# gercap/gr-ofdm_tools

Hardware: AMD Instinct MI355X
Metric: IQ Msamples/s Welch-PSD (4096-pt, 50% ovlp) (higher is better)
Workload: dtype f32; 1 GPU; C2: 2^28-sample complex64 stream, 4096-pt Hann Welch, 50% overlap, detrend constant, density; nfft=4096, noverlap=2048, window=hann, samples_per_gpu=268435456, segments_per_gpu=131071, parallelism=single GPU

## Files before the change

gr-ofdm_tools_amd/csrc/abi_route.hip:

```cpp
#include "abi_state.h"


namespace {
constexpr long long kFdMinSegments = 8;

const W4096Variant kVariants[] = {
    {"dpp", launch_welch_tuned4096_dpp, tuned4096_blocks_per_cu_dpp, 8, false},
    {"pipe", launch_welch_tuned4096_pipe, tuned4096_blocks_per_cu_pipe, 16, false},
    {"ws", launch_welch_tuned4096_ws, tuned4096_blocks_per_cu_ws, 20, true, true},
};
const W4096Variant *variant_by_tag(const char *tag) {
    for (const auto &v : kVariants)
        if (!strcmp(v.tag, tag)) return &v;
    return &kVariants[0];
}
const W4096Variant *w4096_variant(int step, bool fd_ok, const std::string &want) {
    const W4096Variant *const dpp = variant_by_tag("dpp"), *const pipe = variant_by_tag("pipe"), *const ws = variant_by_tag("ws");
    const W4096Variant *pick = (step == 2048) ? (fd_ok ? ws : pipe) : dpp;
    if (!want.empty())
        for (const auto &v : kVariants)
            if (want == v.tag) pick = &v;
    if (pick->fd && !fd_ok) pick = pipe;
    if (pick != dpp && step != 2048) pick = dpp;
    return pick;
}

const char *const kRecipeKernelName[] = {"welch_generic", "welch4096", "csd4096", "csd4096ws", "welch16k", "welch16k1x",
                                         "welch16k1x_half", "seg", "segws", "seg_padded", "anyfft"};

int table_bpc(const OccupancyKey &k) {
    switch (k.kern) {
        case RK_W4096: return !strcmp(k.variant, "ws") ? 2 : 4;
        case RK_CSD4096: return 3;
        case RK_CSD4096WS: return 1;
        case RK_SEGWS: return k.nfft == 1024 ? 8 : 4;
        case RK_SEG: {
            const int tpw = k.nfft == 256 ? 4 : (k.nfft == 512 ? 2 : 1), wpt = k.nfft <= 1024 ? 1 : k.nfft / 1024;
            return 4 * (k.seg_wps4 ? 4 : 3) * tpw / wpt;
        }
        case RK_SEGPAD:
            return k.nfft == 1024 ? 16 : (k.nperseg * 4 == k.nfft ? 8 : (k.seg_kind == 0 ? 6 : 8));
        case RK_W16K: case RK_W16K1X: case RK_W16K1X_HALF: return k.nfft == 8192 && !k.half_ws ? 2 : 1;
        default: return 0;
    }
}

int generic_wg_for(int cu_count, int nfft, long long nseg, int nstreams) {
    const size_t lds = generic_lds_bytes(nfft);
    long long occ = (long long)(160 * 1024 / lds);
    const long long tocc = 2048 / generic_threads_for(nfft);
    if (occ > tocc) occ = tocc;
    if (occ < 1) occ = 1;
    if (occ > 4) occ = 4;
    long long w = ((long long)cu_count * occ + nstreams - 1) / nstreams;
    if (w > nseg) w = nseg;
    if (w < 1) w = 1;
    return (int)w;
}
}

namespace oth {
const char *const kAnyKindName[] = {"none", "direct", "twolevel", "bluestein", "bluestein2"};

bool w4096_variant_known(const char *tag) {
    for (const auto &v : kVariants)
        if (!strcmp(tag, v.tag)) return true;
    return false;
}

int runtime_bpc(const OccupancyKey &k) {
    switch (k.kern) {
        case RK_W4096: return variant_by_tag(k.variant)->blocks_per_cu();
        case RK_CSD4096: return csd4096_blocks_per_cu();
        case RK_CSD4096WS: return csd4096ws_blocks_per_cu();
// ... 232 lines not shown
```

gr-ofdm_tools_amd/csrc/abi_state.h:

```cpp
#pragma once
#include "../../include/ofdm_tools_hip.h"
#include "oth_internal.h"
#include "abi_barrier.h"

#include <algorithm>
#include <cmath>
#include <cstdio>
#include <cstdlib>
#include <cstring>
#include <map>
#include <mutex>
#include <new>
#include <string>
#include <vector>

using namespace oth;

struct oth_ctx {
    int device = 0;
    hipStream_t stream = nullptr;
    bool own_stream = false;
    int cu_count = 256;
    std::string err;
    std::string name;
    bool timing = false;
    std::vector<std::pair<hipEvent_t, hipEvent_t>> events;
    std::vector<std::pair<hipEvent_t, hipEvent_t>> free_events;
    double total_ms = 0.0;
    uint64_t launches = 0;
    std::map<int, float2 *> twiddles;
    float *sink = nullptr;
    double *acc4 = nullptr;
    unsigned *queue = nullptr;
    unsigned *done_count = nullptr;
    std::recursive_mutex mu;
    bool queue_clean = false;
    int queue_used = 0;
    unsigned char *scratch = nullptr;
    size_t scratch_cap = 0;
    std::vector<int> bounds_host;
    int *d_bounds = nullptr;
    int *h_bounds = nullptr;
    size_t bounds_cap = 0;
    hipEvent_t bounds_ev = nullptr;
};

struct AnyTables {
    AnyShape sh{};
    const float2 *tw = nullptr;
    float2 *chirp = nullptr;
    float2 *midtab = nullptr;
    float2 *ws = nullptr;
    size_t ws_cap = 0;
    float4 *mean = nullptr;
    size_t mean_cap = 0;
};

struct oth_plan {
    oth_ctx *ctx = nullptr;
    int nfft = 0, nperseg = 0, noverlap = 0, step = 0, detrend = 0, scaling = 0, fftshift = 0, trim = 0;
    int db = 0, kernel = OTH_KERNEL_AUTO, sched = OTH_SCHED_DYNAMIC;
    double fs = 1.0, scale = 1.0;
    float *d_win = nullptr;
    const float2 *d_tw = nullptr;
    float4 *d_fd = nullptr;
    float4 *d_fd1x = nullptr;
    float2 *d_pilot = nullptr;
    size_t pilot_cap = 0;
    bool fast_detrend = false;
    bool rect_window = false;
    float *d_partial = nullptr;
    size_t partial_cap = 0;
    float *d_reduce = nullptr;
    size_t reduce_cap = 0;
    float *d_out = nullptr;
    size_t out_cap = 0;
    static constexpr int kOutRing = 4;
    float *h_out = nullptr;
    unsigned *h_seq = nullptr;
    uint64_t out_ticket[kOutRing] = {0, 0, 0, 0};
    uint64_t out_nseg[kOutRing] = {0, 0, 0, 0};
    uint64_t next_out_ticket = 1;
    bool pilot_launch = false;
    std::string last_recipe;
    float2 *d_stage = nullptr;
    size_t stage_cap = 0;
    float *d_sum = nullptr;
    float *d_wpm = nullptr;
    uint64_t nseg_total = 0;
    size_t carry = 0;
    float2 *d_stream = nullptr;
    size_t stream_cap = 0;
    std::string tune_variant;
    int tune_sched = -1, tune_chunk = 0, tune_tail = 0;
    void *h_ring[4] = {nullptr, nullptr, nullptr, nullptr};
    size_t h_ring_cap[4] = {0, 0, 0, 0};
    hipEvent_t h_ring_ev[4] = {nullptr, nullptr, nullptr, nullptr};
    unsigned h_ring_next = 0;
    AnyTables any;
    std::mutex exec_mu;
    int hostwait = 0;
    int average = OTH_AVERAGE_MEAN;
    float *d_rows = nullptr;
    size_t rows_cap = 0;
    float *d_med = nullptr;
    size_t med_cap = 0;
    unsigned *d_msel = nullptr;
    size_t msel_cap = 0;
    AnyTables rows_any;
    long long bias_nseg = 0;
    double bias = 1.0;
};

struct oth_chain {
    oth_ctx *ctx = nullptr;
    int nfft = 0, fftshift = 0, epilogue = 0, keep_n = 1, count = 1;
    float *d_win = nullptr;
    const float2 *d_tw = nullptr;
    float2 *d_buf = nullptr;
    size_t buf_cap = 0;
    size_t leftover = 0;
    float *d_rows = nullptr;
    size_t rows_cap = 0;
// ... 228 lines not shown
```

gr-ofdm_tools_amd/csrc/abi_welch.hip:

```cpp
#include "abi_state.h"

#include <sched.h>
#include <time.h>

namespace {
bool window_spectrum(const std::vector<float> &w, int n, int band, std::vector<double> &re, std::vector<double> &im) {
    re.assign(n, 0.0);
    im.assign(n, 0.0);
    double s2 = 0.0;
    for (int i = 0; i < n; ++i) {
        re[i] = (double)w[i];
        s2 += (double)w[i] * (double)w[i];
    }
    host_fft_pow2(re, im);
    for (int k = band; k < n - band; ++k)
        if (re[k] * re[k] + im[k] * im[k] > 1e-10 * s2) return false;
    return true;
}

bool window_spectrum_table(const std::vector<float> &w, std::vector<float> &fd) {
    std::vector<double> re, im;
    if (!window_spectrum(w, 4096, 256, re, im)) return false;
    fd.resize(4 * 256);
    for (int t = 0; t < 256; ++t) {
// ... 4 lines not shown
        fd[4 * t + 3] = (float)im[k + 3840];
    }
    return true;
}

bool window_spectrum_table_seg(const std::vector<float> &w, int n, std::vector<float> &fd) {
    const int R = n / 256, Q = 16 / R;
    std::vector<double> re, im;
    if (!window_spectrum(w, n, 256, re, im)) return false;
    fd.assign((size_t)4 * (n / 16) * Q, 0.f);
    for (int t = 0; t < n / 16; ++t) {
        const int k0 = t / R, j = t % R;
        for (int m = 0; m < Q; ++m) {
            const int lo = k0 + 16 * (j + R * m), hi = lo + 256 * (R - 1);
            float *o = &fd[4 * ((size_t)Q * t + m)];
            o[0] = (float)re[lo];
            o[1] = (float)im[lo];
            o[2] = (float)re[hi];
            o[3] = (float)im[hi];
        }
    }
    return true;
}

bool window_spectrum_table_16k(const std::vector<float> &w, int n, std::vector<float> &fd) {
    const int F = n / 4096;
    std::vector<double> re, im;
    if (!window_spectrum(w, n, 256 * F, re, im)) return false;
    fd.assign((size_t)4 * 256 * F, 0.f);
    for (int tid = 0; tid < 256 * F; ++tid) {
        const int kp = tid >> 8, k0 = (tid >> 4) & 15, k1 = tid & 15;
        const int lo = kp + F * (k0 + 16 * k1), hi = kp + F * (k0 + 16 * k1 + 3840);
        fd[4 * tid] = (float)re[lo];
        fd[4 * tid + 1] = (float)im[lo];
        fd[4 * tid + 2] = (float)re[hi];
        fd[4 * tid + 3] = (float)im[hi];
    }
    return true;
}

bool window_spectrum_table_1x(const std::vector<float> &w, int n, std::vector<float> &fd) {
    std::vector<double> re, im;
    if (!window_spectrum(w, n, 16, re, im)) return false;
    fd.assign((size_t)4 * (n / 16), 0.f);
    for (int k0 = 0; k0 < 16; ++k0) {
        const int lo = n == 16384 ? 64 * k0 : 64 * (k0 >> 1) + 32 * (k0 & 1);
        const int hi = n == 16384 ? 64 * k0 + 63 : 64 * (k0 >> 1) + 32 * (k0 & 1) + 31;
        fd[4 * lo] = (float)re[k0];
        fd[4 * lo + 1] = (float)im[k0];
        const int kh = n - 16 + k0;
        fd[4 * hi + 2] = (float)(-im[kh]);
        fd[4 * hi + 3] = (float)re[kh];
    }
    return true;
}

int segments(const oth_plan *p, size_t nsamples, long long *nseg) {
    if (nsamples < (size_t)p->nperseg) return OTH_ERR_INVALID;
    *nseg = (long long)((nsamples - (size_t)p->noverlap) / (size_t)p->step);
    return OTH_OK;
}

int run_average(oth_plan *p, const float2 *x, const float2 *y, size_t nsamples, int nstreams, size_t stride,
                long long *nseg_out, int *W_out, int *layout_out) {
    oth_ctx *c = p->ctx;
    long long nseg = 0;
    if (segments(p, nsamples, &nseg) != OTH_OK)
        return fail(c, OTH_ERR_INVALID, "input shorter than nperseg");
    const bool csd = (y != nullptr);
    LaunchRecipe r;
    const char *why = "";
    if (int rrc = resolve_recipe(shape_of(p), csd, nseg, nstreams, c->cu_count, runtime_bpc, &r, &why))
        return fail(c, rrc, why);
    p->last_recipe = recipe_text(r, p->nfft);
    int rc = ensure(c, &p->d_partial, &p->partial_cap, sizeof(float) * (size_t)nstreams * r.W * r.nch * p->nfft);
    {
        const int groups = std::max(kReduceGroups, finalize_row_groups(p->nfft, r.W, r.nch));
        if (!rc) rc = ensure(c, &p->d_reduce, &p->reduce_cap, sizeof(float) * (size_t)nstreams * groups * r.nch * p->nfft);
    }
    if (rc) return rc;
    const float4 *fd_tab = r.form == 2 ? (r.use_fd1x ? p->d_fd1x : p->d_fd) : nullptr;
    const float2 *pilot = nullptr;
    if (r.pilot == 1) {
        rc = ensure(c, &p->d_pilot, &p->pilot_cap, sizeof(float2) * 2 * kPilotProbes * (size_t)nstreams);
        if (rc) return rc;
        HIPCHK(c, launch_pilot_mean(x, csd ? y : nullptr, stride, p->nperseg, p->step, nseg, nstreams, p->d_pilot, c->stream));
        pilot = p->d_pilot;
    }
    unsigned *queue = nullptr;
    if (r.tickets) {
        queue = c->queue;
        if (!c->queue_clean) HIPCHK(c, hipMemsetAsync(c->queue, 0, sizeof(unsigned) * 64, c->stream));
        c->queue_clean = false;
        c->queue_used = nstreams;
    }
    if (r.kern == RK_ANY && r.any_onewg) {
        Timed tm(c);
        for (int st = 0; st < nstreams; ++st) {
            W32kArgs a{};
            a.x = x + (size_t)st * stride;
            a.first = 0, a.step = p->step, a.nseg = nseg;
            a.win = p->d_win, a.tw = p->any.tw;
            a.partial = p->d_partial + (size_t)st * r.W * p->nfft;
            a.detrend = p->detrend != OTH_DETREND_NONE;
            a.front = p->nfft == 65536, a.wpm = p->d_wpm;
            HIPCHK(c, launch_welch32k(a, r.W, c->stream));
// ... 5 lines not shown
                         p->detrend != OTH_DETREND_NONE, nseg, p->d_partial + (size_t)st * r.W * r.nch * p->nfft, r.W, nullptr, 0,
                         1.0f, 0, p->tune_variant == "anycov");
            if (rc) return rc;
        }
    } else if (r.kern == RK_SEG || r.kern == RK_SEGWS || r.kern == RK_SEGPAD) {
        SegArgs g{};
        g.x = x;
        g.stream_stride = stride;
        g.nstreams = nstreams;
        g.win = p->d_win;
        g.tw = p->d_tw;
        g.first = 0;
        g.step = p->step;
        g.nseg = nseg;
        g.detrend = p->detrend;
        g.chain = 0;
        g.partial = p->d_partial;
        g.wg_per_stream = r.W;
        g.sched = r.sched;
        g.chunk = r.chunk;
        g.tail_chunk = r.tail_chunk;
        g.nbig = r.nbig;
        g.queue = queue;
        g.fd = fd_tab;
        g.pilot = pilot;
        Timed tm(c);
        switch (r.kern) {
            case RK_SEGPAD: HIPCHK(c, launch_seg_padded(p->nfft, p->nperseg, g, r.seg_kind, c->stream)); break;
            case RK_SEGWS: HIPCHK(c, launch_segws(p->nfft, g, r.seg_det, c->stream)); break;
            default: HIPCHK(c, launch_seg(p->nfft, g, r.seg_kind, r.seg_wps4, c->stream)); break;
        }
    } else {
        WelchArgs a;
        a.x = x;
        a.y = y;
        a.win = p->d_win;
        a.tw = p->d_tw;
        a.partial = p->d_partial;
        a.nseg = nseg;
        a.stream_stride = stride;
        a.nperseg = p->nperseg;
        a.step = p->step;
        a.detrend = p->detrend;
        a.wg_per_stream = r.W;
        a.nstreams = nstreams;
        a.sched = r.sched;
        a.chunk = r.chunk;
        a.tail_chunk = r.tail_chunk;
        a.nbig = r.nbig;
        a.queue = queue;
        a.fd = fd_tab;
        a.pilot = pilot;
        a.pilot_inline = r.pilot == 2 ? 1 : 0;
        Timed tm(c);
        switch (r.kern) {
            case RK_W4096: HIPCHK(c, r.variant->launch(a, c->stream)); break;
            case RK_CSD4096WS: HIPCHK(c, launch_csd_tuned4096ws(a, c->stream)); break;
            case RK_CSD4096: HIPCHK(c, launch_csd_tuned4096(a, c->stream)); break;
            case RK_W16K1X_HALF:
                HIPCHK(c, r.half_ws ? launch_welch_tuned8kws(a, c->stream) : launch_welch_tuned16k1x_half(p->nfft, a, c->stream));
                break;
            case RK_W16K1X: HIPCHK(c, launch_welch_tuned16k1x(p->nfft, a, r.x1_window, r.x1_plain, c->stream)); break;
            case RK_W16K: HIPCHK(c, launch_welch_tuned16k(p->nfft, a, c->stream)); break;
            default: HIPCHK(c, launch_welch_generic(p->nfft, a, c->stream)); break;
        }
    }
    *nseg_out = nseg;
    *W_out = r.W;
    *layout_out = r.layout;
    return OTH_OK;
}

int finalize_and_rearm(oth_ctx *c, FinalizeArgs &f, int nstreams) {
    f.queue_reset = nullptr;
    f.queue_n = 0;
    if (!c->queue_clean && c->queue_used > 0) {
        f.queue_reset = c->queue;
        f.queue_n = c->queue_used;
    }
    HIPCHK(c, launch_finalize(f, nstreams, c->stream));
    if (f.queue_reset) {
        c->queue_clean = true;
        c->queue_used = 0;
    }
    return OTH_OK;
}

FinalizeArgs finalize_args(const oth_plan *p, int W, int layout, int nch) {
    FinalizeArgs f{};
    f.partial = p->d_partial;
    f.scratch = p->d_reduce;
    f.W = W;
    f.nfft = p->nfft;
    f.nch = nch;
    f.layout = layout;
    f.l1 = p->any.sh.L1, f.l2 = p->any.sh.L2;
    return f;
}

template <typename P> hipError_t upload_table(oth_ctx *c, P **dst, const std::vector<float> &h) {
    hipError_t e = hipMalloc(dst, sizeof(float) * h.size());
    if (e == hipSuccess) e = hipMemcpyAsync(*dst, h.data(), sizeof(float) * h.size(), hipMemcpyHostToDevice, c->stream);
    return e;
}

double median_bias(long long n) {
// ... 108 lines not shown
    if (trim_bins < 0 || 2 * trim_bins >= nfft) return fail(c, OTH_ERR_INVALID, "trim_bins out of range");
    if (!(fs > 0.0)) return fail(c, OTH_ERR_INVALID, "fs must be positive");
    if (use_device(c)) return OTH_ERR_HIP;
    oth_plan *p = new (std::nothrow) oth_plan();
    if (!p) return fail(c, OTH_ERR_NOMEM, "host allocation failed");
    p->ctx = c;
    p->nfft = nfft;
    p->nperseg = nperseg;
    p->noverlap = noverlap;
    p->step = nperseg - noverlap;
    p->detrend = detrend;
    p->fast_detrend = fast_detrend;
    p->scaling = scaling;
    p->fs = fs;
    p->fftshift = fftshift != 0;
    p->trim = trim_bins;
    if (const char *e = getenv("OTH_W4096_VARIANT")) p->tune_variant = e;
    if (const char *e = getenv("OTH_W4096_SCHED")) p->tune_sched = atoi(e);
    if (const char *e = getenv("OTH_W4096_CHUNK")) p->tune_chunk = atoi(e);
    if (const char *e = getenv("OTH_W4096_TAIL")) p->tune_tail = atoi(e);
    if (const char *e = getenv("OTH_PILOT_LAUNCH")) p->pilot_launch = atoi(e) != 0;
    if (const char *e = getenv("OTH_HOSTWAIT")) p->hostwait = !strcmp(e, "sync") ? 1 : 0;
    std::vector<float> w(nfft, 0.f);
    double s1 = 0.0, s2 = 0.0;
    p->rect_window = true;
    for (int i = 0; i < nperseg; ++i) {
        w[i] = window ? window[i] : 1.0f;
        if (w[i] != 1.0f) p->rect_window = false;
        s1 += (double)w[i];
        s2 += (double)w[i] * (double)w[i];
    }
    switch (scaling) {
        case OTH_SCALE_DENSITY: p->scale = 1.0 / (fs * s2); break;
        case OTH_SCALE_OVER_N2: p->scale = 1.0 / ((double)nfft * (double)nfft); break;
        case OTH_SCALE_SPECTRUM: p->scale = 1.0 / (s1 * s1); break;
        default: p->scale = 1.0;
    }
    int rc = any_route ? any_tables_init(c, nfft, &p->any) : get_twiddles(c, nfft, &p->d_tw);
    if (rc) {
        delete p;
        return rc;
    }
    hipError_t e = hipMalloc(&p->d_win, sizeof(float) * nfft);
    if (e == hipSuccess) e = hipMalloc(&p->d_sum, sizeof(float) * nfft);
    if (e == hipSuccess) e = hipMemcpyAsync(p->d_win, w.data(), sizeof(float) * nfft, hipMemcpyHostToDevice, c->stream);
    if (e == hipSuccess) e = hipMemsetAsync(p->d_sum, 0, sizeof(float) * nfft, c->stream);
    std::vector<float> fd;
    if (e == hipSuccess && detrend == OTH_DETREND_CONSTANT &&
        ((nfft == 4096 && nperseg == 4096 && window_spectrum_table(w, fd)) ||
         (nfft == 2048 && nperseg == 2048 && window_spectrum_table_seg(w, nfft, fd)) ||
         ((nfft == 8192 || nfft == 16384) && nperseg == nfft && window_spectrum_table_16k(w, nfft, fd)))) {
        e = upload_table(c, &p->d_fd, fd);
    }
    std::vector<float> fd1x;
    if (e == hipSuccess && detrend == OTH_DETREND_CONSTANT && (nfft == 16384 || nfft == 8192) && nperseg == nfft &&
        window_spectrum_table_1x(w, nfft, fd1x)) {
        e = upload_table(c, &p->d_fd1x, fd1x);
    }
    std::vector<float> wpm;
    if (e == hipSuccess && any_route && nfft == 65536 && nperseg == 65536) {
        wpm.resize(65536);
        for (int n = 0; n < 32768; ++n) {
            wpm[n] = (float)((double)w[n] + (double)w[n + 32768]);
            wpm[32768 + n] = (float)((double)w[n] - (double)w[n + 32768]);
        }
        e = upload_table(c, &p->d_wpm, wpm);
    }
    if (e == hipSuccess) e = hipStreamSynchronize(c->stream);
    if (e != hipSuccess) {
        oth_plan_destroy(p);
        return fail(c, OTH_ERR_HIP, std::string("plan setup: ") + hipGetErrorString(e));
    }
    *out = p;
    return OTH_OK;
    OTH_CATCH(c)
}

int oth_plan_destroy(oth_plan *p) {
    OTH_TRY
    CtxGuard guard_(p ? p->ctx : nullptr);
    if (!p) return OTH_OK;
    oth_ctx *c = p->ctx;
    hipSetDevice(c->device);
    hipStreamSynchronize(c->stream);
    if (p->d_win) hipFree(p->d_win);
    if (p->d_wpm) hipFree(p->d_wpm);
    if (p->d_fd) hipFree(p->d_fd);
    if (p->d_fd1x) hipFree(p->d_fd1x);
    if (p->d_pilot) hipFree(p->d_pilot);
    if (p->d_partial) hipFree(p->d_partial);
    if (p->d_reduce) hipFree(p->d_reduce);
    if (p->d_out) hipFree(p->d_out);
    if (p->h_out) hipHostFree(p->h_out);
    if (p->h_seq) hipHostFree(p->h_seq);
    if (p->d_stage) hipFree(p->d_stage);
    if (p->d_sum) hipFree(p->d_sum);
    if (p->d_stream) hipFree(p->d_stream);
    any_tables_free(p->any);
    any_tables_free(p->rows_any);
    if (p->d_rows) hipFree(p->d_rows);
    if (p->d_med) hipFree(p->d_med);
    if (p->d_msel) hipFree(p->d_msel);
    for (int i = 0; i < 4; ++i) {
        if (p->h_ring[i]) hipHostFree(p->h_ring[i]);
        if (p->h_ring_ev[i]) hipEventDestroy(p->h_ring_ev[i]);
    }
    delete p;
    return OTH_OK;
    OTH_CATCH((p ? p->ctx : nullptr))
}

int oth_plan_set_output_db(oth_plan *p, int enable) {
    OTH_TRY
    CtxGuard guard_(p ? p->ctx : nullptr);
    if (!p) return fail(nullptr, OTH_ERR_INVALID, "plan is NULL");
    p->db = enable != 0;
    return OTH_OK;
    OTH_CATCH((p ? p->ctx : nullptr))
}

int oth_plan_set_kernel(oth_plan *p, int which) {
    OTH_TRY
    CtxGuard guard_(p ? p->ctx : nullptr);
    if (!p) return fail(nullptr, OTH_ERR_INVALID, "plan is NULL");
    if (which < OTH_KERNEL_AUTO || which > OTH_KERNEL_TUNED) return fail(p->ctx, OTH_ERR_INVALID, "unknown kernel id");
    p->kernel = which;
    return OTH_OK;
    OTH_CATCH((p ? p->ctx : nullptr))
}

int oth_plan_set_schedule(oth_plan *p, int which) {
    OTH_TRY
    CtxGuard guard_(p ? p->ctx : nullptr);
    if (!p) return fail(nullptr, OTH_ERR_INVALID, "plan is NULL");
    if (which < OTH_SCHED_CONTIGUOUS || which > OTH_SCHED_DYNAMIC) return fail(p->ctx, OTH_ERR_INVALID, "unknown schedule");
    p->sched = which;
    return OTH_OK;
    OTH_CATCH((p ? p->ctx : nullptr))
}

int oth_plan_set_tuning(oth_plan *p, const char *variant, int sched, int chunk, int tail_chunk) {
    OTH_TRY
    CtxGuard guard_(p ? p->ctx : nullptr);
    if (!p) return fail(nullptr, OTH_ERR_INVALID, "plan is NULL");
    if (sched < -1 || sched > OTH_SCHED_DYNAMIC || chunk < 0 || tail_chunk < 0)
        return fail(p->ctx, OTH_ERR_INVALID, "bad tuning value");
    if (variant && *variant) {
        bool known = !strcmp(variant, "seg3") || !strcmp(variant, "seg4") || !strcmp(variant, "segws") ||
                     !strcmp(variant, "csd1") ||
                     !strcmp(variant, "fd") || !strcmp(variant, "td") ||
                     !strcmp(variant, "plaunch") ||
                     !strcmp(variant, "16k4") || !strcmp(variant, "16kplain") ||
                     !strcmp(variant, "8kws") || !strcmp(variant, "8k1role") ||
                     !strcmp(variant, "anycov") ||
                     !strcmp(variant, "r16");
        known = known || w4096_variant_known(variant);
        if (!known) return fail(p->ctx, OTH_ERR_UNSUPPORTED, std::string("unknown kernel build: ") + variant);
    }
    p->tune_variant = variant ? variant : "";
    p->tune_sched = sched;
    p->tune_chunk = chunk;
    p->tune_tail = tail_chunk;
    return OTH_OK;
    OTH_CATCH((p ? p->ctx : nullptr))
}

int oth_plan_set_hostwait(oth_plan *p, int mode) {
    OTH_TRY
    CtxGuard guard_(p ? p->ctx : nullptr);
    if (!p) return fail(nullptr, OTH_ERR_INVALID, "plan is NULL");
    if (mode != OTH_HOSTWAIT_POLL && mode != OTH_HOSTWAIT_SYNC) return fail(p->ctx, OTH_ERR_INVALID, "unknown host-wait mode");
    p->hostwait = mode;
    return OTH_OK;
    OTH_CATCH((p ? p->ctx : nullptr))
}

int oth_plan_out_len(oth_plan *p, int *n) {
    OTH_TRY
    CtxGuard guard_(p ? p->ctx : nullptr);
    if (!p || !n) return fail(p ? p->ctx : nullptr, OTH_ERR_INVALID, "bad argument");
    *n = p->nfft - 2 * p->trim;
    return OTH_OK;
    OTH_CATCH((p ? p->ctx : nullptr))
}

int oth_plan_set_average(oth_plan *p, int mode) {
    OTH_TRY
    CtxGuard guard_(p ? p->ctx : nullptr);
    if (!p) return fail(nullptr, OTH_ERR_INVALID, "plan is NULL");
    if (mode != OTH_AVERAGE_MEAN && mode != OTH_AVERAGE_MEDIAN) return fail(p->ctx, OTH_ERR_INVALID, "unknown average mode");
    if (p->nseg_total || p->carry)
        return fail(p->ctx, OTH_ERR_STATE, "an accumulation is in progress (oth_welch_finalize or oth_welch_reset first)");
    p->average = mode;
    return OTH_OK;
    OTH_CATCH((p ? p->ctx : nullptr))
}

int oth_welch_segments_dev(oth_plan *p, const void *iq_dev, size_t nsamples, float *rows_dev, uint64_t capacity_rows,
                           uint64_t *nseg_out) {
    OTH_TRY
    CtxGuard guard_(p ? p->ctx : nullptr);
    if (!p) return fail(nullptr, OTH_ERR_INVALID, "plan is NULL");
    oth_ctx *c = p->ctx;
    if (!iq_dev || !rows_dev) return fail(c, OTH_ERR_INVALID, "bad argument");
// ... 495 lines not shown
```

gr-ofdm_tools_amd/csrc/fft4096.hip.h:

```cpp
#pragma once
#include "fft_lds.hip.h"
#include "oth_internal.h"

static_assert(oth::kPilotProbes == 8, "load_pilot() (fft_lds.hip.h) adds eight probe means");

namespace oth {
namespace {

constexpr int T4 = 256;
constexpr int RS = 272;
constexpr int LDS_X = 16 * RS;
constexpr int LDS_RED = 16;
constexpr size_t LDS_BYTES = (LDS_X + LDS_RED) * sizeof(float2);

constexpr float C1 = 0.92387953251128674f;
constexpr float S1 = 0.38268343236508977f;
constexpr float RH = 0.70710678118654752f;

__device__ __forceinline__ float2 mul_w1(float2 a) { return make_float2(fmaf(a.x, C1, a.y * S1), fmaf(a.y, C1, -a.x * S1)); }
__device__ __forceinline__ float2 mul_w2(float2 a) { return make_float2((a.x + a.y) * RH, (a.y - a.x) * RH); }
__device__ __forceinline__ float2 mul_w3(float2 a) { return make_float2(fmaf(a.x, S1, a.y * C1), fmaf(a.y, S1, -a.x * C1)); }
__device__ __forceinline__ float2 mul_w4(float2 a) { return make_float2(a.y, -a.x); }
__device__ __forceinline__ float2 mul_w6(float2 a) { return make_float2((a.y - a.x) * RH, -(a.x + a.y) * RH); }
__device__ __forceinline__ float2 mul_w9(float2 a) { return make_float2(-fmaf(a.x, C1, a.y * S1), fmaf(a.x, S1, -a.y * C1)); }
// ... 153 lines not shown
    const I rest = nseg - nbig * chunk;
    return nbig + (rest + tail_chunk - 1) / tail_chunk;
}
template <class I> __device__ __forceinline__ void chunk_range_of(I nseg, I nbig, int chunk, int tail_chunk, I c, I &sb, I &se) {
    if (c < nbig) {
        sb = c * chunk;
        se = sb + chunk;
    } else {
        sb = nbig * chunk + (c - nbig) * tail_chunk;
        se = sb + tail_chunk < nseg ? sb + tail_chunk : nseg;
    }
}

__device__ __forceinline__ void prio_latency() { __builtin_amdgcn_s_setprio(2); }
__device__ __forceinline__ void prio_compute() { __builtin_amdgcn_s_setprio(0); }

__device__ __forceinline__ void lds_barrier() { asm volatile("s_waitcnt lgkmcnt(0)\n\ts_barrier" ::: "memory"); }

template <int STRIDE>
__device__ __forceinline__ void scatter_pow16(const float2 (&v)[16], float2 *out, float2 p1, float2 p4) {
    float2 wj[4], wi[4];
    wj[1] = p1;
    wi[1] = p4;
    asm volatile("" : "+v"(wj[1].x), "+v"(wj[1].y), "+v"(wi[1].x), "+v"(wi[1].y));
    wj[2] = cmul(wj[1], wj[1]);
    wj[3] = cmul(wj[2], wj[1]);
    wi[2] = cmul(wi[1], wi[1]);
    wi[3] = cmul(wi[2], wi[1]);
    out[0] = v[0];
#pragma unroll
    for (int k = 1; k < 16; ++k) {
        const int i = k >> 2, j = k & 3;
        const float2 w = (i == 0) ? wj[j] : ((j == 0) ? wi[i] : cmul(wi[i], wj[j]));
        out[STRIDE * k] = cmul(v[r16(k)], w);
    }
}

template <int STRIDE>
__device__ __forceinline__ void scatter_pow16_six(const float2 (&v)[16], float2 *out, float2 p1, float2 p2, float2 p3, float2 p4,
                                                  float2 p8, float2 p12) {
    float2 wj[4], wi[4];
    wj[1] = p1, wj[2] = p2, wj[3] = p3;
    wi[1] = p4, wi[2] = p8, wi[3] = p12;
    asm volatile("" : "+v"(wj[1].x), "+v"(wj[1].y), "+v"(wj[2].x), "+v"(wj[2].y), "+v"(wj[3].x), "+v"(wj[3].y));
    out[0] = v[0];
#pragma unroll
    for (int k = 1; k < 16; ++k) {
        const int i = k >> 2, j = k & 3;
        const float2 w = (i == 0) ? wj[j] : ((j == 0) ? wi[i] : cmul(wi[i], wj[j]));
        out[STRIDE * k] = cmul(v[r16(k)], w);
    }
}

__device__ __forceinline__ void wave_lds_sync() {
    __builtin_amdgcn_fence(__ATOMIC_RELEASE, "wavefront");
    __builtin_amdgcn_wave_barrier();
    __builtin_amdgcn_fence(__ATOMIC_ACQUIRE, "wavefront");
}

template <int CTRL> __device__ __forceinline__ float dpp_add(float v) {
    const int x = __builtin_amdgcn_update_dpp(0, __float_as_int(v), CTRL, 0xF, 0xF, true);
    return v + __int_as_float(x);
}

__device__ __forceinline__ float wave_total(float v) {
    v = dpp_add<0xB1>(v);
    v = dpp_add<0x4E>(v);
    v = dpp_add<0x141>(v);
    v = dpp_add<0x140>(v);
    const int i = __float_as_int(v);
    return __int_as_float(__builtin_amdgcn_readlane(i, 0)) + __int_as_float(__builtin_amdgcn_readlane(i, 16)) +
           __int_as_float(__builtin_amdgcn_readlane(i, 32)) + __int_as_float(__builtin_amdgcn_readlane(i, 48));
}

__device__ __forceinline__ float wave_total_lane63(float v) {
    v = dpp_add<0xB1>(v);
    v = dpp_add<0x4E>(v);
    v = dpp_add<0x141>(v);
    v = dpp_add<0x140>(v);
    asm("s_nop 1\n\tv_add_f32_dpp %0, %0, %0 row_bcast:15 row_mask:0xa bank_mask:0xf" : "+v"(v));
    asm("s_nop 1\n\tv_add_f32_dpp %0, %0, %0 row_bcast:31 row_mask:0xc bank_mask:0xf" : "+v"(v));
    return v;
}

struct PilotProbes {
    float2 v[kPilotProbes];
};
__device__ __forceinline__ PilotProbes inline_pilot_load(const float2 *xb, long long nseg, int step, int t) {
    PilotProbes r;
#pragma unroll
    for (int k = 0; k < kPilotProbes; ++k) {
        const long long seg = ((nseg - 1) * k) / (kPilotProbes - 1);
        const float2 *src = xb + (size_t)__builtin_amdgcn_readfirstlane((int)seg) * (size_t)step + 512 * k;
        r.v[k] = src[(unsigned)t];
    }
    return r;
}
__device__ __forceinline__ void inline_pilot_store(const PilotProbes &r, int t, float2 *slot) {
#pragma unroll
    for (int k = 0; k < kPilotProbes; ++k) {
        const float2 s = make_float2(wave_total_lane63(r.v[k].x), wave_total_lane63(r.v[k].y));
        if ((t & 63) == 63) slot[4 * k + (t >> 6)] = s;
    }
}
__device__ __forceinline__ float2 inline_pilot_value(const float2 *slot) {
    float2 q[kPilotProbes];
// ... 12 lines not shown
```

gr-ofdm_tools_amd/csrc/oth_internal.h:

```cpp
#pragma once
#include <hip/hip_runtime.h>
#include <stdint.h>
#include <stddef.h>

namespace oth {

constexpr int kPilotProbes = 8;

struct WelchArgs {
    const float2 *x;
    const float2 *y;
    const float *win;
    const float2 *tw;
    float *partial;
    long long nseg;
    size_t stream_stride;
    int nperseg;
    int step;
    int detrend;
    int wg_per_stream;
    int nstreams;
    int sched;
    int chunk;
    int tail_chunk;
    long long nbig;
    unsigned *queue;
    const float4 *fd;
    const float2 *pilot;
    int pilot_inline;
};

struct SegArgs {
    const float2 *x;
    size_t stream_stride;
    int nstreams;
    const float *win;
    const float2 *tw;
    const float4 *fd;
    const float2 *pilot;
    long long first;
    long long step;
    long long nseg;
    int detrend;
    int chain;
    float *partial;
    int acc_mode;
    long long acc_end;
    float l2;
    float *rows;
    long long store_from;
    int epilogue;
    float scale;
    int fftshift;
    int wg_per_stream;
    int sched;
    int chunk;
    int tail_chunk;
    long long nbig;
    unsigned *queue;
};

struct PgramArgs {
    const float2 *x;
    const float *win;
    const float2 *tw;
    float *rows;
    long long first_vec;
    long long nrows;
    int keep_n;
    int fftshift;
    int epilogue;
    float scale;
};

constexpr int kReduceGroups = 16;
inline int finalize_row_groups(int nfft, int W, int nch) {
    if (nch != 1 || nfft > 1024 || (nfft % 256) != 0 || W < 1024) return 0;
    return 65536 / nfft;
}

struct FinalizeArgs {
    const float *partial;
// ... 211 lines not shown
```

gr-ofdm_tools_amd/csrc/welch4096ws.hip:

```cpp

#include <type_traits>
#include "fft4096.hip.h"

namespace oth {
namespace {

constexpr int TWS = 512;
constexpr int WS_RED = 32;
constexpr int WS_CTRL = 16;
constexpr size_t WS_WIN_BYTES = 256 * 2 * sizeof(float4);
constexpr size_t WS_LDS_BYTES = (2 * LDS_X + WS_RED) * sizeof(float2) + WS_CTRL * sizeof(int) + WS_WIN_BYTES;

constexpr int WS_PAL = 2, WS_PAC = 0, WS_PAS = WS_PAL, WS_PBL = 2;
constexpr int WS_PBC = 1;

enum { ITEM_STOP = 0, ITEM_DATA = 1, ITEM_BUBBLE = 2 };

template <bool DETREND, bool PILOT = false>
__global__ __launch_bounds__(TWS, 4) void welch4096ws_kernel(WelchArgs p) {
    static_assert(DETREND || !PILOT, "the pilot belongs to the detrend");
    extern __shared__ __attribute__((aligned(16))) unsigned char smem[];
    float2 *img = reinterpret_cast<float2 *>(smem);
    float2 *red = img + 2 * LDS_X;
    int *ctrl = reinterpret_cast<int *>(red + WS_RED);

    const int tid = threadIdx.x;
    const bool producer = tid < 256;
    const int t = tid & 255;
    const int hi = t >> 4, lo = t & 15;
    const int wave = t >> 6;
    const int wg = blockIdx.x, W = p.wg_per_stream, stream = blockIdx.y;
    const float2 *xb = p.x + (size_t)stream * p.stream_stride;
    const int sched = p.sched;
    const long long nchunks = sched ? chunk_count(p) : 1;

    const int w1 = hi * 17 + lo, r1 = hi * RS + lo, w2 = hi * RS + lo, r2 = hi * RS + lo * 17;

    if (producer) {
        float win[8];
        float4 *wl = reinterpret_cast<float4 *>(ctrl + WS_CTRL) + t;
#pragma unroll
        for (int a = 0; a < 8; ++a) win[a] = p.win[256 * a + t];
        wl[0] = make_float4(p.win[256 * 8 + t], p.win[256 * 9 + t], p.win[256 * 10 + t], p.win[256 * 11 + t]);
        wl[256] = make_float4(p.win[256 * 12 + t], p.win[256 * 13 + t], p.win[256 * 14 + t], p.win[256 * 15 + t]);
        const float2 b1 = p.tw[t], b2 = p.tw[2 * t], b3 = p.tw[3 * t], b4 = p.tw[4 * t], b8 = p.tw[8 * t],
                     b12 = p.tw[(12 * t) & 4095];
        float2 kw[8], nxt[8];
        float2 prev_new = make_float2(0.f, 0.f);
        float2 pv = make_float2(0.f, 0.f);
        if (PILOT && !p.pilot_inline) pv = load_pilot(p.pilot, stream);
        int it = 0;
        unsigned ticket = 0;
        using std::false_type;
        using std::true_type;
        using mid = std::integral_constant<int, 0>;
        using head = std::integral_constant<int, 1>;
        using none = std::integral_constant<int, 2>;

        auto uni = [](int v) { return __builtin_amdgcn_readfirstlane(v); };
        auto load_chunk_head = [&](int first_seg) {
            const float2 *xs = xb + (size_t)uni(first_seg) * 2048;
#pragma unroll
            for (int j = 0; j < 4; ++j) {
                const float2 *xj = xs + 512 * j;
                kw[2 * j] = *(xj + (unsigned)t);
                kw[2 * j + 1] = *(xj + ((unsigned)t + 256u));
            }
#pragma unroll
            for (int j = 0; j < 4; ++j) {
                const float2 *xj = xs + 2048 + 512 * j;
                nxt[2 * j] = load_once(xj + (unsigned)t);
                nxt[2 * j + 1] = load_once(xj + ((unsigned)t + 256u));
            }
        };
        auto step_end = [&](int item) {
            if (t == 0) ctrl[it & 1] = item;
            lds_barrier();
            ++it;
        };
        auto item = [&](auto first_, auto mode_, int s, int nsb, bool publish) {
            constexpr bool FIRST = decltype(first_)::value;
            constexpr int MODE = decltype(mode_)::value;
            const int q = it & 1;
            float2 *lx = img + q * LDS_X;
            __builtin_amdgcn_s_setprio(WS_PAL);
            float2 v[16];
            float2 sumf = make_float2(0.f, 0.f), sum = make_float2(0.f, 0.f);
            const float4 wa = wl[0], wb = wl[256];
            const float wh[8] = {wa.x, wa.y, wa.z, wa.w, wb.x, wb.y, wb.z, wb.w};
            if (FIRST) {
#pragma unroll
                for (int a = 0; a < 8; ++a) {
                    if (PILOT) kw[a] = csub(kw[a], pv);
                    sumf = cadd(sumf, kw[a]);
                    kw[a] = make_float2(kw[a].x * win[a], kw[a].y * win[a]);
                }
            }
#pragma unroll
            for (int a = 0; a < 8; ++a) {
                const float2 r = PILOT ? csub(nxt[a], pv) : nxt[a];
                v[a] = kw[a];
                v[8 + a] = make_float2(r.x * wh[a], r.y * wh[a]);
                if (MODE == 0) kw[a] = make_float2(r.x * win[a], r.y * win[a]);
                sum = cadd(sum, r);
            }
            if (sched == 2 && t == 0) {
                if (FIRST) ticket = atomicAdd(p.queue + stream, 1u);
                if (publish) ctrl[4] = (int)ticket;
            }
            const float2 *xn = xb + (size_t)uni(s + 2) * 2048;
            auto load_next = [&]() {
#pragma unroll
                for (int j = 0; j < 4; ++j) {
                    const float2 *xj = xn + 512 * j;
                    nxt[2 * j] = load_once(xj + (unsigned)t);
                    nxt[2 * j + 1] = load_once(xj + ((unsigned)t + 256u));
                }
            };
            if (MODE == 0) {
                load_next();
            } else if (MODE == 1) {
                load_chunk_head(nsb);
            }
            if (DETREND) {
                sum.x = wave_total_lane63(sum.x);
                sum.y = wave_total_lane63(sum.y);
                float2 other = prev_new;
                if (FIRST) other = make_float2(wave_total_lane63(sumf.x), wave_total_lane63(sumf.y));
                if ((t & 63) == 63) red[q * 8 + wave] = cadd(sum, other);
                prev_new = sum;
            }
            __builtin_amdgcn_s_setprio(WS_PAC);
            dft16(v);
            __builtin_amdgcn_s_setprio(WS_PAS);
            scatter_pow16_six<RS>(v, lx + w1, b1, b2, b3, b4, b8, b12);
            step_end(ITEM_DATA);
        };

        int cur = 0, sb = 0, se = 0;
        auto range = [&](int c, int &b, int &e) {
            long long lb, le;
            chunk_range(p, c, lb, le);
            b = uni((int)lb);
            e = uni((int)le);
        };
        auto open_chunk = [&](int c) -> bool {
            cur = c;
            if (sched) {
                if (cur >= nchunks) return false;
                range(cur, sb, se);
                return true;
            }
            sb = uni((int)((p.nseg * wg) / W));
            se = uni((int)((p.nseg * (wg + 1)) / W));
            return sb < se;
        };
        bool have = open_chunk(sched ? wg : 0);
        if (have) load_chunk_head(sb);
        if (PILOT && p.pilot_inline) {
            const bool own = sched == 0 && have;
            const PilotProbes probes = inline_pilot_load(own ? xb + (size_t)sb * 2048 : xb, own ? (long long)(se - sb) : p.nseg, 2048, t);
            inline_pilot_store(probes, t, img + LDS_X);
            lds_barrier();
            pv = inline_pilot_value(img + LDS_X);
        }
        while (have) {
            const int n = se - sb;
            int ncur = 0;
            if (n >= 2) {
                item(true_type{}, mid{}, sb, 0, n == 2);
                int s = sb + 1;
                if (s < se - 1) item(false_type{}, mid{}, s++, 0, true);
                for (; s + 1 < se - 1; s += 2) {
                    item(false_type{}, mid{}, s, 0, false);
                    item(false_type{}, mid{}, s + 1, 0, false);
                }
                if (s < se - 1) item(false_type{}, mid{}, s, 0, false);
                ncur = (sched == 1) ? cur + W : W + uni(ctrl[4]);
                int nsb = 0, nse = 0;
                const bool have_next = sched && ncur < nchunks;
                if (have_next) {
                    range(ncur, nsb, nse);
                    item(false_type{}, head{}, se - 1, nsb, false);
                    cur = ncur;
                    sb = nsb;
                    se = nse;
                    continue;
                }
                item(false_type{}, none{}, se - 1, 0, false);
                break;
            }
            item(true_type{}, none{}, sb, 0, true);
            if (sched == 0) break;
            if (sched == 2) {
                step_end(ITEM_BUBBLE);
                ncur = W + uni(ctrl[4]);
            } else {
                ncur = cur + W;
            }
            have = open_chunk(ncur);
            if (have) load_chunk_head(sb);
        }
        step_end(ITEM_STOP);
    } else {
        float2 tw2[16];
#pragma unroll
        for (int k = 1; k < 16; ++k) tw2[k] = p.tw[16 * lo * k];
        float4 fw = make_float4(0.f, 0.f, 0.f, 0.f);
        if (DETREND) fw = p.fd[t];
        float acc[16];
#pragma unroll
        for (int k = 0; k < 16; ++k) acc[k] = 0.f;
        float2 v[16];
        float2 mean = make_float2(0.f, 0.f);
        int it = 0;
        auto next_item = [&]() -> int {
            __builtin_amdgcn_s_setprio(WS_PBL);
            lds_barrier();
            const int q = it & 1;
            const float2 *lq = img + q * LDS_X;
            const int kind = ctrl[q];
            const float2 h0 = red[q * 8], h1 = red[q * 8 + 1], h2 = red[q * 8 + 2], h3 = red[q * 8 + 3];
            dft16_from_lds<17>(v, lq + r1, [] { __builtin_amdgcn_s_setprio(WS_PBC); });
            if (DETREND) {
                const float2 tot = cadd(cadd(h0, h1), cadd(h2, h3));
                mean = make_float2(tot.x * (1.0f / 4096.0f), tot.y * (1.0f / 4096.0f));
            }
            ++it;
            return kind;
        };
        if (PILOT && p.pilot_inline) lds_barrier();
        int item = next_item();
        for (;;) {
            while (item == ITEM_BUBBLE) item = next_item();
            if (item == ITEM_STOP) break;
            float2 *lx = img + ((it & 1) ^ 1) * LDS_X;
            __builtin_amdgcn_s_setprio(WS_PBL);
            lx[w2] = v[r16(0)];
#pragma unroll
            for (int k1 = 1; k1 < 16; ++k1) lx[w2 + k1 * 17] = cmul(v[r16(k1)], tw2[k1]);
            wave_lds_sync();
            dft16_from_lds<1>(v, lx + r2, [] { __builtin_amdgcn_s_setprio(WS_PBC); });
            if (DETREND) {
                v[r16(0)] = make_float2(v[r16(0)].x - (mean.x * fw.x - mean.y * fw.y),
                                        v[r16(0)].y - (mean.x * fw.y + mean.y * fw.x));
                v[r16(15)] = make_float2(v[r16(15)].x - (mean.x * fw.z - mean.y * fw.w),
                                         v[r16(15)].y - (mean.x * fw.w + mean.y * fw.z));
            }
#pragma unroll
            for (int k2 = 0; k2 < 16; ++k2) {
                const float2 X = v[r16(k2)];
                acc[k2] = fmaf(X.x, X.x, fmaf(X.y, X.y, acc[k2]));
            }
            item = next_item();
        }
        float *dst = p.partial + ((size_t)stream * W + wg) * 4096;
#pragma unroll
        for (int k2 = 0; k2 < 16; ++k2) dst[256 * k2 + t] = acc[k2];
    }
}

}

int tuned4096_blocks_per_cu_ws() {
    static int cached = 0;
    if (cached) return cached;
    int n = 0;
    if (hipOccupancyMaxActiveBlocksPerMultiprocessor(&n, welch4096ws_kernel<true, false>, TWS, WS_LDS_BYTES) != hipSuccess || n < 1)
        n = 1;
    return cached = n;
}

hipError_t launch_welch_tuned4096_ws(const WelchArgs &a, hipStream_t s) {
    const dim3 grid(a.wg_per_stream, a.nstreams);
    static bool armed[64] = {};
    int dev = 0;
    if (hipGetDevice(&dev) != hipSuccess || dev < 0 || dev >= 64) dev = 63, armed[63] = false;
    bool &big_lds = armed[dev];
    if (!big_lds) {
        hipError_t e = hipSuccess;
        for (const void *fn : {reinterpret_cast<const void *>(welch4096ws_kernel<true, true>),
                               reinterpret_cast<const void *>(welch4096ws_kernel<true, false>),
                               reinterpret_cast<const void *>(welch4096ws_kernel<false, false>)})
            if (e == hipSuccess) e = hipFuncSetAttribute(fn, hipFuncAttributeMaxDynamicSharedMemorySize, (int)WS_LDS_BYTES);
        if (e != hipSuccess) return e;
        big_lds = true;
    }
    if (a.detrend && (a.pilot || a.pilot_inline))
        hipLaunchKernelGGL((welch4096ws_kernel<true, true>), grid, dim3(TWS), WS_LDS_BYTES, s, a);
    else if (a.detrend)
        hipLaunchKernelGGL((welch4096ws_kernel<true, false>), grid, dim3(TWS), WS_LDS_BYTES, s, a);
    else
        hipLaunchKernelGGL((welch4096ws_kernel<false, false>), grid, dim3(TWS), WS_LDS_BYTES, s, a);
    return hipGetLastError();
}

}
```

Baseline: 441,900 Msamples/s.

## Add complementary-window ws kernel variant reusing overlapped half and stored twiddle powers

Detects windows whose two halves sum to one (periodic Hann) and launches a specialised producer path for them. That path keeps only the raw overlapped half and derives the second-half window as 1-w through an fma, which frees eight window registers. It spends those registers on preloaded twiddle powers so the scatter needs fewer complex multiplies, and it pins the consumer's twiddle and fd registers with asm constraints. The trade-off is a second kernel instantiation, an exact float tolerance check that can misroute near-complementary windows, and possible register-pressure changes.

```diff
diff --git a/gr-ofdm_tools_amd/csrc/abi_route.hip b/gr-ofdm_tools_amd/csrc/abi_route.hip
--- a/gr-ofdm_tools_amd/csrc/abi_route.hip
+++ b/gr-ofdm_tools_amd/csrc/abi_route.hip
@@ -19,7 +19,7 @@
     const W4096Variant *pick = (step == 2048) ? (fd_ok ? ws : pipe) : dpp;
     if (!want.empty())
         for (const auto &v : kVariants)
-            if (want == v.tag) pick = &v;
+            if (want == v.tag || (want == "wsgen" && !strcmp(v.tag, "ws"))) pick = &v;
     if (pick->fd && !fd_ok) pick = pipe;
     if (pick != dpp && step != 2048) pick = dpp;
     return pick;
diff --git a/gr-ofdm_tools_amd/csrc/abi_state.h b/gr-ofdm_tools_amd/csrc/abi_state.h
--- a/gr-ofdm_tools_amd/csrc/abi_state.h
+++ b/gr-ofdm_tools_amd/csrc/abi_state.h
@@ -69,6 +69,7 @@
     size_t pilot_cap = 0;
     bool fast_detrend = false;
     bool rect_window = false;
+    bool compl_window = false;
     float *d_partial = nullptr;
     size_t partial_cap = 0;
     float *d_reduce = nullptr;
diff --git a/gr-ofdm_tools_amd/csrc/abi_welch.hip b/gr-ofdm_tools_amd/csrc/abi_welch.hip
--- a/gr-ofdm_tools_amd/csrc/abi_welch.hip
+++ b/gr-ofdm_tools_amd/csrc/abi_welch.hip
@@ -80,6 +80,12 @@
         fd[4 * hi + 2] = (float)(-im[kh]);
         fd[4 * hi + 3] = (float)re[kh];
     }
+    return true;
+}
+
+bool window_is_complementary(const std::vector<float> &w, int n) {
+    for (int i = 0; i < n / 2; ++i)
+        if (!(std::fabs((double)w[i] + (double)w[i + n / 2] - 1.0) <= 1.1920928955078125e-07)) return false;
     return true;
 }
 
@@ -191,6 +197,7 @@
         a.fd = fd_tab;
         a.pilot = pilot;
         a.pilot_inline = r.pilot == 2 ? 1 : 0;
+        a.compl_win = p->compl_window && p->tune_variant != "wsgen" ? 1 : 0;
         Timed tm(c);
         switch (r.kern) {
             case RK_W4096: HIPCHK(c, r.variant->launch(a, c->stream)); break;
@@ -405,6 +412,7 @@
          ((nfft == 8192 || nfft == 16384) && nperseg == nfft && window_spectrum_table_16k(w, nfft, fd)))) {
         e = upload_table(c, &p->d_fd, fd);
     }
+    p->compl_window = nfft == 4096 && nperseg == 4096 && window_is_complementary(w, nfft);
     std::vector<float> fd1x;
     if (e == hipSuccess && detrend == OTH_DETREND_CONSTANT && (nfft == 16384 || nfft == 8192) && nperseg == nfft &&
         window_spectrum_table_1x(w, nfft, fd1x)) {
@@ -503,6 +511,7 @@
                      !strcmp(variant, "csd1") ||
                      !strcmp(variant, "fd") || !strcmp(variant, "td") ||
                      !strcmp(variant, "plaunch") ||
+                     !strcmp(variant, "wsgen") ||
                      !strcmp(variant, "16k4") || !strcmp(variant, "16kplain") ||
                      !strcmp(variant, "8kws") || !strcmp(variant, "8k1role") ||
                      !strcmp(variant, "anycov") ||
diff --git a/gr-ofdm_tools_amd/csrc/fft4096.hip.h b/gr-ofdm_tools_amd/csrc/fft4096.hip.h
--- a/gr-ofdm_tools_amd/csrc/fft4096.hip.h
+++ b/gr-ofdm_tools_amd/csrc/fft4096.hip.h
@@ -229,6 +229,27 @@
     }
 }
 
+__host__ __device__ constexpr int pow16_slot(int k) { return k - 5 - (k >> 2) + 1; }
+template <int STRIDE, int NM>
+__device__ __forceinline__ void scatter_pow16_stored(const float2 (&v)[16], float2 *out, float2 p1, float2 p2, float2 p3, float2 p4,
+                                                     float2 p8, float2 p12, const float2 (&pm)[NM]) {
+    float2 wj[4], wi[4];
+    wj[1] = p1, wj[2] = p2, wj[3] = p3;
+    wi[1] = p4, wi[2] = p8, wi[3] = p12;
+    asm volatile("" : "+v"(wj[1].x), "+v"(wj[1].y), "+v"(wj[2].x), "+v"(wj[2].y), "+v"(wj[3].x), "+v"(wj[3].y));
+    out[0] = v[0];
+#pragma unroll
+    for (int k = 1; k < 16; ++k) {
+        const int i = k >> 2, j = k & 3;
+        float2 w;
+        if (i == 0) w = wj[j];
+        else if (j == 0) w = wi[i];
+        else if (pow16_slot(k) < NM) w = pm[pow16_slot(k) < NM ? pow16_slot(k) : 0];
+        else w = cmul(wi[i], wj[j]);
+        out[STRIDE * k] = cmul(v[r16(k)], w);
+    }
+}
+
 __device__ __forceinline__ void wave_lds_sync() {
     __builtin_amdgcn_fence(__ATOMIC_RELEASE, "wavefront");
     __builtin_amdgcn_wave_barrier();
diff --git a/gr-ofdm_tools_amd/csrc/oth_internal.h b/gr-ofdm_tools_amd/csrc/oth_internal.h
--- a/gr-ofdm_tools_amd/csrc/oth_internal.h
+++ b/gr-ofdm_tools_amd/csrc/oth_internal.h
@@ -28,6 +28,7 @@
     const float4 *fd;
     const float2 *pilot;
     int pilot_inline;
+    int compl_win;
 };
 
 struct SegArgs {
diff --git a/gr-ofdm_tools_amd/csrc/welch4096ws.hip b/gr-ofdm_tools_amd/csrc/welch4096ws.hip
--- a/gr-ofdm_tools_amd/csrc/welch4096ws.hip
+++ b/gr-ofdm_tools_amd/csrc/welch4096ws.hip
@@ -16,8 +16,13 @@
 
 enum { ITEM_STOP = 0, ITEM_DATA = 1, ITEM_BUBBLE = 2 };
 
-template <bool DETREND, bool PILOT = false>
-__global__ __launch_bounds__(TWS, 4) void welch4096ws_kernel(WelchArgs p) {
+#ifndef OTH_WS_COMPL_POWERS
+#define OTH_WS_COMPL_POWERS 13
+#endif
+constexpr int WS_COMPL_POWERS = OTH_WS_COMPL_POWERS;
+
+template <bool DETREND, bool PILOT, bool COMPL>
+__device__ __forceinline__ void welch4096ws_body(const WelchArgs &p) {
     static_assert(DETREND || !PILOT, "the pilot belongs to the detrend");
     extern __shared__ __attribute__((aligned(16))) unsigned char smem[];
     float2 *img = reinterpret_cast<float2 *>(smem);
@@ -37,14 +42,23 @@
     const int w1 = hi * 17 + lo, r1 = hi * RS + lo, w2 = hi * RS + lo, r2 = hi * RS + lo * 17;
 
     if (producer) {
-        float win[8];
+        float win[COMPL ? 1 : 8];
         float4 *wl = reinterpret_cast<float4 *>(ctrl + WS_CTRL) + t;
-#pragma unroll
-        for (int a = 0; a < 8; ++a) win[a] = p.win[256 * a + t];
-        wl[0] = make_float4(p.win[256 * 8 + t], p.win[256 * 9 + t], p.win[256 * 10 + t], p.win[256 * 11 + t]);
-        wl[256] = make_float4(p.win[256 * 12 + t], p.win[256 * 13 + t], p.win[256 * 14 + t], p.win[256 * 15 + t]);
+        constexpr int WROW = COMPL ? 0 : 8;
+        if constexpr (!COMPL) {
+#pragma unroll
+            for (int a = 0; a < 8; ++a) win[a] = p.win[256 * a + t];
+        }
+        wl[0] = make_float4(p.win[256 * WROW + t], p.win[256 * (WROW + 1) + t], p.win[256 * (WROW + 2) + t], p.win[256 * (WROW + 3) + t]);
+        wl[256] = make_float4(p.win[256 * (WROW + 4) + t], p.win[256 * (WROW + 5) + t], p.win[256 * (WROW + 6) + t],
+                              p.win[256 * (WROW + 7) + t]);
         const float2 b1 = p.tw[t], b2 = p.tw[2 * t], b3 = p.tw[3 * t], b4 = p.tw[4 * t], b8 = p.tw[8 * t],
                      b12 = p.tw[(12 * t) & 4095];
+        float2 bm[WS_COMPL_POWERS - 6 > 0 && COMPL ? WS_COMPL_POWERS - 6 : 1];
+        if constexpr (COMPL) {
+#pragma unroll
+            for (int k = 0; k < WS_COMPL_POWERS - 6; ++k) bm[k] = p.tw[((5 + k + k / 3) * t) & 4095];
+        }
         float2 kw[8], nxt[8];
         float2 prev_new = make_float2(0.f, 0.f);
         float2 pv = make_float2(0.f, 0.f);
@@ -83,6 +97,7 @@
             constexpr int MODE = decltype(mode_)::value;
             const int q = it & 1;
             float2 *lx = img + q * LDS_X;
+            if constexpr (COMPL) asm volatile("; item %0 %1" ::"n"((int)FIRST), "n"(MODE));
             __builtin_amdgcn_s_setprio(WS_PAL);
             float2 v[16];
             float2 sumf = make_float2(0.f, 0.f), sum = make_float2(0.f, 0.f);
@@ -93,16 +108,22 @@
                 for (int a = 0; a < 8; ++a) {
                     if (PILOT) kw[a] = csub(kw[a], pv);
                     sumf = cadd(sumf, kw[a]);
-                    kw[a] = make_float2(kw[a].x * win[a], kw[a].y * win[a]);
+                    if constexpr (!COMPL) kw[a] = make_float2(kw[a].x * win[a], kw[a].y * win[a]);
                 }
             }
 #pragma unroll
             for (int a = 0; a < 8; ++a) {
                 const float2 r = PILOT ? csub(nxt[a], pv) : nxt[a];
-                v[a] = kw[a];
-                v[8 + a] = make_float2(r.x * wh[a], r.y * wh[a]);
-                if (MODE == 0) kw[a] = make_float2(r.x * win[a], r.y * win[a]);
-                sum = cadd(sum, r);
+                if constexpr (COMPL) {
+                    v[a] = make_float2(kw[a].x * wh[a], kw[a].y * wh[a]);
+                    v[8 + a] = make_float2(fmaf(-r.x, wh[a], r.x), fmaf(-r.y, wh[a], r.y));
+                    if (MODE == 0) kw[a] = r;
+                } else {
+                    v[a] = kw[a];
+                    v[8 + a] = make_float2(r.x * wh[a], r.y * wh[a]);
+                    if (MODE == 0) kw[a] = make_float2(r.x * win[a], r.y * win[a]);
+                }
+                sum = (COMPL && a == 0) ? r : cadd(sum, r);
             }
             if (sched == 2 && t == 0) {
                 if (FIRST) ticket = atomicAdd(p.queue + stream, 1u);
@@ -133,7 +154,8 @@
             __builtin_amdgcn_s_setprio(WS_PAC);
             dft16(v);
             __builtin_amdgcn_s_setprio(WS_PAS);
-            scatter_pow16_six<RS>(v, lx + w1, b1, b2, b3, b4, b8, b12);
+            if constexpr (COMPL) scatter_pow16_stored<RS>(v, lx + w1, b1, b2, b3, b4, b8, b12, bm);
+            else scatter_pow16_six<RS>(v, lx + w1, b1, b2, b3, b4, b8, b12);
             step_end(ITEM_DATA);
         };
 
@@ -213,6 +235,13 @@
         for (int k = 0; k < 16; ++k) acc[k] = 0.f;
         float2 v[16];
         float2 mean = make_float2(0.f, 0.f);
+        asm volatile("s_waitcnt vmcnt(0)"
+                     : "+v"(tw2[1].x), "+v"(tw2[1].y), "+v"(tw2[2].x), "+v"(tw2[2].y), "+v"(tw2[3].x), "+v"(tw2[3].y), "+v"(tw2[4].x),
+                       "+v"(tw2[4].y), "+v"(tw2[5].x), "+v"(tw2[5].y), "+v"(tw2[6].x), "+v"(tw2[6].y), "+v"(tw2[7].x), "+v"(tw2[7].y));
+        asm volatile("" : "+v"(tw2[8].x), "+v"(tw2[8].y), "+v"(tw2[9].x), "+v"(tw2[9].y), "+v"(tw2[10].x), "+v"(tw2[10].y),
+                          "+v"(tw2[11].x), "+v"(tw2[11].y), "+v"(tw2[12].x), "+v"(tw2[12].y), "+v"(tw2[13].x), "+v"(tw2[13].y));
+        asm volatile("" : "+v"(tw2[14].x), "+v"(tw2[14].y), "+v"(tw2[15].x), "+v"(tw2[15].y), "+v"(fw.x), "+v"(fw.y), "+v"(fw.z),
+                          "+v"(fw.w));
         int it = 0;
         auto next_item = [&]() -> int {
             __builtin_amdgcn_s_setprio(WS_PBL);
@@ -260,6 +289,15 @@
     }
 }
 
+template <bool DETREND, bool PILOT = false>
+__global__ __launch_bounds__(TWS, 4) void welch4096ws_kernel(WelchArgs p) {
+    welch4096ws_body<DETREND, PILOT, false>(p);
+}
+template <bool DETREND, bool PILOT = false>
+__global__ __launch_bounds__(TWS, 4) void welch4096ws_compl_kernel(WelchArgs p) {
+    welch4096ws_body<DETREND, PILOT, true>(p);
+}
+
 }
 
 int tuned4096_blocks_per_cu_ws() {
@@ -281,12 +319,20 @@
         hipError_t e = hipSuccess;
         for (const void *fn : {reinterpret_cast<const void *>(welch4096ws_kernel<true, true>),
                                reinterpret_cast<const void *>(welch4096ws_kernel<true, false>),
-                               reinterpret_cast<const void *>(welch4096ws_kernel<false, false>)})
+                               reinterpret_cast<const void *>(welch4096ws_kernel<false, false>),
+                               reinterpret_cast<const void *>(welch4096ws_compl_kernel<true, true>),
+                               reinterpret_cast<const void *>(welch4096ws_compl_kernel<true, false>),
+                               reinterpret_cast<const void *>(welch4096ws_compl_kernel<false, false>)})
             if (e == hipSuccess) e = hipFuncSetAttribute(fn, hipFuncAttributeMaxDynamicSharedMemorySize, (int)WS_LDS_BYTES);
         if (e != hipSuccess) return e;
         big_lds = true;
     }
-    if (a.detrend && (a.pilot || a.pilot_inline))
+    const bool pilot = a.detrend && (a.pilot || a.pilot_inline);
+    if (a.compl_win) {
+        if (pilot) hipLaunchKernelGGL((welch4096ws_compl_kernel<true, true>), grid, dim3(TWS), WS_LDS_BYTES, s, a);
+        else if (a.detrend) hipLaunchKernelGGL((welch4096ws_compl_kernel<true, false>), grid, dim3(TWS), WS_LDS_BYTES, s, a);
+        else hipLaunchKernelGGL((welch4096ws_compl_kernel<false, false>), grid, dim3(TWS), WS_LDS_BYTES, s, a);
+    } else if (pilot)
         hipLaunchKernelGGL((welch4096ws_kernel<true, true>), grid, dim3(TWS), WS_LDS_BYTES, s, a);
     else if (a.detrend)
         hipLaunchKernelGGL((welch4096ws_kernel<true, false>), grid, dim3(TWS), WS_LDS_BYTES, s, a);
```

Measured after the change: 452,200 Msamples/s, median of 6. 1.02x the previous value.
